# SavaRobotics/FoundationPose

Hardware: AMD Instinct MI355X
Metric: pose-hypotheses/sec (render+refine+score), 252 hyp x 160x160 (higher is better)
Workload: dtype f16

## Files before the change

### foundationpose_amd/csrc/crop.hip

```cpp
#include "common.h"

__device__ __forceinline__ int round_snapped(double x) {
  double f = floor(x), t = x - f;
  if (fabs(t - 0.5) < 1e-4) {
    long long fi = (long long)f;
    return (int)((fi & 1) ? fi + 1 : fi);
  }
  return (int)floor(x + 0.5);
}

__device__ __forceinline__ float frame_at(const float *img, int H, int W, int C, int y, int x, int c) {
  return (y >= 0 && y < H && x >= 0 && x < W) ? img[((size_t)y * W + x) * C + c] : 0.f;
}

__device__ __forceinline__ void crop_observed_px(const CropArgs &a, int b, float mesh_diameter) {
  const int p = blockIdx.x * blockDim.x + threadIdx.x;
  const float *T = a.tf + (size_t)b * 9;
  const float *pose = a.poses + (size_t)b * 16;
  const int H = a.H, W = a.W;
  __shared__ double s_aff[4];
  if (threadIdx.x == 0) {
    const double sx0 = T[0], tx0 = T[2], sy0 = T[4], ty0 = T[5];
    s_aff[0] = (1.0 / sx0) * W / (W - 1.0);
    s_aff[1] = (-tx0 / sx0) * W / (W - 1.0) - 0.5;
    s_aff[2] = (1.0 / sy0) * H / (H - 1.0);
    s_aff[3] = (-ty0 / sy0) * H / (H - 1.0) - 0.5;
  }
  __syncthreads();
  if (p >= a.Ho * a.Wo) return;
  const int j = p / a.Wo, i = p - j * a.Wo;
  const double sx = T[0], tx = T[2], sy = T[4], ty = T[5];
  const double ax = s_aff[0], bx = s_aff[1], ay = s_aff[2], by = s_aff[3];
  const double xd = ax * i + bx, yd = ay * j + by;
  const float x = (float)xd, y = (float)yd;

  float rgb[3];
  {
    float x0f = floorf(x), y0f = floorf(y);
    int x0 = (int)x0f, y0 = (int)y0f, x1 = x0 + 1, y1 = y0 + 1;
    float x1f = x0f + 1.f, y1f = y0f + 1.f;
    float nw = (x1f - x) * (y1f - y), ne = (x - x0f) * (y1f - y), sw = (x1f - x) * (y - y0f), se = (x - x0f) * (y - y0f);
#pragma unroll
    for (int c = 0; c < 3; ++c) {
      float acc = 0.f;
      acc = __fadd_rn(acc, __fmul_rn(frame_at(a.rgb, H, W, 3, y0, x0, c), nw));
      acc = __fadd_rn(acc, __fmul_rn(frame_at(a.rgb, H, W, 3, y0, x1, c), ne));
      acc = __fadd_rn(acc, __fmul_rn(frame_at(a.rgb, H, W, 3, y1, x0, c), sw));
      acc = __fadd_rn(acc, __fmul_rn(frame_at(a.rgb, H, W, 3, y1, x1, c), se));
      rgb[c] = __fdiv_rn(acc, 255.f);
    }
  }
  const int qx = round_snapped(xd), qy = round_snapped(yd);
  const bool q_in = (qx >= 0 && qx < W && qy >= 0 && qy < H);
  float xyz[3] = {0.f, 0.f, 0.f};
  float invalid_thres;
  if (a.mode == 0) {
    invalid_thres = 0.001f;
    if (q_in) {
#pragma unroll
      for (int c = 0; c < 3; ++c) xyz[c] = a.geom[((size_t)qy * W + qx) * 3 + c];
    }
  } else {
    invalid_thres = 0.1f;
    if (q_in) {
      const double cxp = (sx * qx + tx) * a.Wo / (a.Wo - 1.0) - 0.5;
      const double cyp = (sy * qy + ty) * a.Ho / (a.Ho - 1.0) - 0.5;
      const int pi = round_snapped(cxp), pj = round_snapped(cyp);
      float z = 0.f;
      if (pi >= 0 && pi < a.Wo && pj >= 0 && pj < a.Ho) {
        const int rx = round_snapped(ax * pi + bx), ry = round_snapped(ay * pj + by);
        if (rx >= 0 && rx < W && ry >= 0 && ry < H) z = a.geom[(size_t)ry * W + rx];
      }
      const float fx = (float)a.K[0], fy = (float)a.K[4], cx = (float)a.K[2], cy = (float)a.K[5];
      if (!(z < 0.001f)) {
        xyz[0] = __fdiv_rn(__fmul_rn(__fsub_rn((float)qx, cx), z), fx);
        xyz[1] = __fdiv_rn(__fmul_rn(__fsub_rn((float)qy, cy), z), fy);
        xyz[2] = z;
      }
    }
  }
  const bool invalid = xyz[2] < invalid_thres;
  const float radius = __fdiv_rn(mesh_diameter, 2.f);
  const float inv_r = __fdiv_rn(1.f, radius);
  float o6[6] = {rgb[0], rgb[1], rgb[2], 0.f, 0.f, 0.f};
#pragma unroll
  for (int c = 0; c < 3; ++c) {
    float v = __fsub_rn(xyz[c], pose[c * 4 + 3]);
    if (a.normalize_xyz) {
      v = __fmul_rn(v, inv_r);
      if (invalid || fabsf(v) >= 2.f) v = 0.f;
    }
    o6[3 + c] = v;
  }
  if (a.out_fmt == 0) {
    float *out = (float *)a.out + (size_t)b * 6 * a.Ho * a.Wo;
#pragma unroll
    for (int c = 0; c < 6; ++c) out[(size_t)c * a.Ho * a.Wo + p] = o6[c];
  } else {
    half8 hv;
#pragma unroll
    for (int c = 0; c < 6; ++c) hv[c] = (f16)o6[c];
    hv[6] = (f16)0.f;
    hv[7] = (f16)0.f;
    *reinterpret_cast<half8 *>((f16 *)a.out + ((size_t)b * a.Ho * a.Wo + p) * 8) = hv;
  }
}

__global__ __launch_bounds__(256) void crop_observed_kernel(CropArgs a) { crop_observed_px(a, blockIdx.y, a.mesh_diameter); }

struct CropDiameters {
  float d[FP_TRACK_MAX_OBJECTS];
};
__global__ __launch_bounds__(256) void crop_observed_objects_kernel(CropArgs a, CropDiameters t) { crop_observed_px(a, blockIdx.y, t.d[blockIdx.y]); }

int launch_crop_observed(const CropArgs &a, hipStream_t s) {
  FP_REQUIRE(a.mode == 0 || a.mode == 1, "crop_observed: mode must be 0 (refiner) or 1 (scorer)");
  FP_REQUIRE(a.H > 1 && a.W > 1 && a.Ho > 1 && a.Wo > 1, "crop_observed: degenerate image size");
  if (a.N == 0) return FP_OK;
  dim3 grid((a.Ho * a.Wo + 255) / 256, a.N);
  hipLaunchKernelGGL(crop_observed_kernel, grid, dim3(256), 0, s, a);
  FP_CHECK_HIP(hipGetLastError());
  return FP_OK;
}

int launch_crop_observed_objects(const CropArgs &a, const float *diameter, hipStream_t s) {
  FP_REQUIRE(a.mode == 0 || a.mode == 1, "crop_observed: mode must be 0 (refiner) or 1 (scorer)");
  FP_REQUIRE(a.H > 1 && a.W > 1 && a.Ho > 1 && a.Wo > 1, "crop_observed: degenerate image size");
  FP_REQUIRE(a.N >= 0 && a.N <= FP_TRACK_MAX_OBJECTS, "crop_observed: %d objects in one launch (at most %d)", a.N, FP_TRACK_MAX_OBJECTS);
  if (a.N == 0) return FP_OK;
  CropDiameters t;
  memset(&t, 0, sizeof(t));
  for (int b = 0; b < a.N; ++b) t.d[b] = diameter[b];
  hipLaunchKernelGGL(crop_observed_objects_kernel, dim3((a.Ho * a.Wo + 255) / 256, a.N), dim3(256), 0, s, a, t);
  FP_CHECK_HIP(hipGetLastError());
  return FP_OK;
}

__global__ __launch_bounds__(256) void warp_nearest_kernel(const float *__restrict__ src, size_t src_batch_stride, int Hs, int Ws, int C,
                                                           const float *__restrict__ tf, int Ho, int Wo, float *__restrict__ out) {
  const int b = blockIdx.y;
  const int p = blockIdx.x * blockDim.x + threadIdx.x;
  if (p >= Ho * Wo) return;
  const float *T = tf + (size_t)b * 9;
  const double sx = T[0], tx = T[2], sy = T[4], ty = T[5];
  const double ax = (1.0 / sx) * Ws / (Ws - 1.0), bx = (-tx / sx) * Ws / (Ws - 1.0) - 0.5;
  const double ay = (1.0 / sy) * Hs / (Hs - 1.0), by = (-ty / sy) * Hs / (Hs - 1.0) - 0.5;
  const int j = p / Wo, i = p - j * Wo;
  const int qx = round_snapped(ax * i + bx), qy = round_snapped(ay * j + by);
  const bool in = qx >= 0 && qx < Ws && qy >= 0 && qy < Hs;
  const float *s = src + (size_t)b * src_batch_stride + ((size_t)(in ? qy : 0) * Ws + (in ? qx : 0)) * C;
  float *o = out + (size_t)b * C * Ho * Wo + p;
  for (int c = 0; c < C; ++c) o[(size_t)c * Ho * Wo] = in ? s[c] : 0.f;
}

int launch_warp_nearest(const float *src, int src_batch, int Hs, int Ws, int C, const float *tf, int N, int Ho, int Wo, float *out,
                        hipStream_t s) {
  FP_REQUIRE(Hs > 1 && Ws > 1 && Ho > 0 && Wo > 0 && C > 0, "warp_nearest: degenerate image size");
  FP_REQUIRE(src_batch == 1 || src_batch == N, "warp_nearest: the source batch is 1 (broadcast) or N");
  if (N == 0) return FP_OK;
  dim3 grid((Ho * Wo + 255) / 256, N);
  hipLaunchKernelGGL(warp_nearest_kernel, grid, dim3(256), 0, s, src, src_batch == 1 ? (size_t)0 : (size_t)Hs * Ws * C, Hs, Ws, C, tf, Ho,
                     Wo, out);
  FP_CHECK_HIP(hipGetLastError());
  return FP_OK;
}

__global__ void erode_depth_kernel(const float *__restrict__ depth, int H, int W, int radius, float diff_thres, float ratio_thres,
                                   float zfar, float *__restrict__ out) {
  int w = blockIdx.x * blockDim.x + threadIdx.x, h = blockIdx.y * blockDim.y + threadIdx.y;
  if (w >= W || h >= H) return;
  float d_ori = depth[(size_t)h * W + w];
  float bad = 0.f, total = 0.f;
  for (int u = w - radius; u <= w + radius; ++u) {
    if (u < 0 || u >= W) continue;
    for (int v = h - radius; v <= h + radius; ++v) {
      if (v < 0 || v >= H) continue;
      float cur = depth[(size_t)v * W + u];
      total += 1.f;
      if (cur < 0.001f || cur >= zfar || fabsf(cur - d_ori) > diff_thres) bad += 1.f;
    }
  }
  out[(size_t)h * W + w] = (__fdiv_rn(bad, total) > ratio_thres) ? 0.f : d_ori;
}

__global__ void bilateral_depth_kernel(const float *__restrict__ depth, int H, int W, int radius, float zfar, float sigmaD,
                                       float sigmaR, float *__restrict__ out) {
  int w = blockIdx.x * blockDim.x + threadIdx.x, h = blockIdx.y * blockDim.y + threadIdx.y;
  if (w >= W || h >= H) return;
  float mean_depth = 0.f;
  int num_valid = 0;
  for (int u = w - radius; u <= w + radius; ++u) {
    if (u < 0 || u >= W) continue;
    for (int v = h - radius; v <= h + radius; ++v) {
      if (v < 0 || v >= H) continue;
      float cur = depth[(size_t)v * W + u];
      if (cur >= 0.001f && cur < zfar) {
        num_valid += 1;
        mean_depth = __fadd_rn(mean_depth, cur);
      }
    }
  }
  float res = 0.f;
  if (num_valid > 0) {
    mean_depth = __fdiv_rn(mean_depth, (float)num_valid);
    float dc = depth[(size_t)h * W + w];
    float sum_w = 0.f, sum = 0.f;
    const float den_d = __fmul_rn(__fmul_rn(2.f, sigmaD), sigmaD), den_r = __fmul_rn(__fmul_rn(2.f, sigmaR), sigmaR);
    for (int u = w - radius; u <= w + radius; ++u) {
      if (u < 0 || u >= W) continue;
      for (int v = h - radius; v <= h + radius; ++v) {
        if (v < 0 || v >= H) continue;
        float cur = depth[(size_t)v * W + u];
        if (cur >= 0.001f && cur < zfar && fabsf(cur - mean_depth) < 0.01f) {
          float sp = __fdiv_rn(-(float)((u - w) * (u - w) + (h - v) * (h - v)), den_d);
          float df = __fsub_rn(dc, cur);
          float rg = __fdiv_rn(__fmul_rn(df, df), den_r);
          float wt = expf(__fsub_rn(sp, rg));
          sum_w = __fadd_rn(sum_w, wt);
          sum = __fadd_rn(sum, __fmul_rn(wt, cur));
        }
      }
    }
    if (sum_w > 0.f) res = __fdiv_rn(sum, sum_w);
  }
  out[(size_t)h * W + w] = res;
}

__global__ void depth2xyz_kernel(const float *__restrict__ depth, int H, int W, float fx, float fy, float cx, float cy, float zfar,
                                 float *__restrict__ xyz) {
  int w = blockIdx.x * blockDim.x + threadIdx.x, h = blockIdx.y * blockDim.y + threadIdx.y;
  if (w >= W || h >= H) return;
  float z = depth[(size_t)h * W + w];
  float o[3] = {0.f, 0.f, 0.f};
  if (!(z < 0.001f) && !(z > zfar)) {
    o[0] = __fdiv_rn(__fmul_rn(__fsub_rn((float)w, cx), z), fx);
    o[1] = __fdiv_rn(__fmul_rn(__fsub_rn((float)h, cy), z), fy);
    o[2] = z;
  }
  size_t p = ((size_t)h * W + w) * 3;
  xyz[p] = o[0];
  xyz[p + 1] = o[1];
  xyz[p + 2] = o[2];
}

static dim3 grid2d(int H, int W) { return dim3((W + 31) / 32, (H + 7) / 8); }

int launch_erode(const float *d, int H, int W, int radius, float diff_thres, float ratio_thres, float zfar, float *out, hipStream_t s) {
  hipLaunchKernelGGL(erode_depth_kernel, grid2d(H, W), dim3(32, 8), 0, s, d, H, W, radius, diff_thres, ratio_thres, zfar, out);
  FP_CHECK_HIP(hipGetLastError());
  return FP_OK;
}
int launch_bilateral(const float *d, int H, int W, int radius, float zfar, float sigmaD, float sigmaR, float *out, hipStream_t s) {
  hipLaunchKernelGGL(bilateral_depth_kernel, grid2d(H, W), dim3(32, 8), 0, s, d, H, W, radius, zfar, sigmaD, sigmaR, out);
  FP_CHECK_HIP(hipGetLastError());
  return FP_OK;
}
int launch_depth2xyz(const float *d, int H, int W, const double *K, float zfar, float *xyz, hipStream_t s) {
  hipLaunchKernelGGL(depth2xyz_kernel, grid2d(H, W), dim3(32, 8), 0, s, d, H, W, (float)K[0], (float)K[4], (float)K[2], (float)K[5],
                     zfar, xyz);
  FP_CHECK_HIP(hipGetLastError());
  return FP_OK;
}

#define PF_R 2
#define PF_TW 32
#define PF_TH 8
__global__ __launch_bounds__(PF_TW *PF_TH) void depth_prefilter_kernel(const float *__restrict__ depth, int H, int W, float diff_thres,
                                                                       float ratio_thres, float zfar_e, float zfar_b, float sigmaD, float sigmaR,
                                                                       float fx, float fy, float cx, float cy, float zfar_x,
                                                                       float *__restrict__ out, float *__restrict__ xyz,
                                                                       const unsigned char *__restrict__ rgb_u8, float *__restrict__ rgb_f) {
  constexpr int R = PF_R, RW = PF_TW + 4 * R, RH = PF_TH + 4 * R, EW = PF_TW + 2 * R, EH = PF_TH + 2 * R, NTAP = (2 * R + 1) * (2 * R + 1);
  __shared__ float raw[RH][RW + 1], er[EH][EW + 1], sp_tab[NTAP];
  const float OUTSIDE = -__builtin_inff();
  const int tid = threadIdx.y * PF_TW + threadIdx.x, w0 = blockIdx.x * PF_TW, h0 = blockIdx.y * PF_TH;
  if (tid < NTAP) {
    const int du = tid / (2 * R + 1), dv = tid % (2 * R + 1);
    sp_tab[tid] = __fdiv_rn(-(float)((du - R) * (du - R) + (dv - R) * (dv - R)), __fmul_rn(__fmul_rn(2.f, sigmaD), sigmaD));
  }
  for (int i = tid; i < RH * RW; i += PF_TW * PF_TH) {
    const int r = i / RW, c = i - r * RW, h = h0 - 2 * R + r, w = w0 - 2 * R + c;
    raw[r][c] = (h >= 0 && h < H && w >= 0 && w < W) ? depth[(size_t)h * W + w] : OUTSIDE;
  }
  __syncthreads();
  for (int i = tid; i < EH * EW; i += PF_TW * PF_TH) {
    const int r = i / EW, c = i - r * EW;
// ... 172 lines not shown
```

### foundationpose_amd/csrc/raster.hip

```cpp
#include "common.h"
#include "pose_math.h"
#include <cstdlib>
#include <type_traits>

#define RB_THREADS 1024

__device__ __forceinline__ unsigned ordered_key(float z) {
  unsigned b = __float_as_uint(z);
  return (b & 0x80000000u) ? ~b : (b | 0x80000000u);
}

struct Vtx {
  int X, Y;
  float w, zn;
  bool ok;
};

__device__ __forceinline__ Vtx xform_vertex(const float *__restrict__ pos, int v, const float *M, float hw, float hh) {
  float px = pos[v * 3], py = pos[v * 3 + 1], pz = pos[v * 3 + 2];
  float c0 = fmaf(M[0], px, fmaf(M[1], py, fmaf(M[2], pz, M[3])));
  float c1 = fmaf(M[4], px, fmaf(M[5], py, fmaf(M[6], pz, M[7])));
  float c2 = fmaf(M[8], px, fmaf(M[9], py, fmaf(M[10], pz, M[11])));
  float c3 = fmaf(M[12], px, fmaf(M[13], py, fmaf(M[14], pz, M[15])));
  Vtx o;
// ... 180 lines not shown
  __shared__ float sM[16];
  __shared__ float sP[12];
  const int b = blockIdx.x, grp = blockIdx.y;
  const MeshDev &m = a.mesh;
  const uint2 *gA = recA + (size_t)b * m.V;
  const int f0 = grp * Fg, f1 = min(m.F, f0 + Fg);
  for (int i = threadIdx.x; i < S * 3; i += RB_THREADS) cs[i / 3][i % 3] = 0;
  if constexpr (FUSED) {
    if (threadIdx.x == 0) {
      clip_matrix(a, b, a.poses + (size_t)b * 16, sM);
      for (int i = 0; i < 12; ++i) sP[i] = a.poses[(size_t)b * 16 + i];
    }
    __syncthreads();
    for (int v = threadIdx.x; v < m.V; v += RB_THREADS) {
      const VtxRecords q = vertex_records(a, a.mesh, v, sM, sP);
      cl_ldsA[v] = q.a;
      if ((v / RB_THREADS) % G == grp) {
        const size_t r = (size_t)b * m.V + v;
        recC[r] = q.c;
        recA[r] = q.a;
        recB[2 * r] = q.b0;
        recB[2 * r + 1] = q.b1;
      }
    }
  } else if (lds_verts) {
    for (int i = threadIdx.x; i < m.V; i += RB_THREADS) cl_ldsA[i] = gA[i];
  }
  __syncthreads();
  auto getA = [&](int i) -> uint2 { return (FUSED || lds_verts) ? cl_ldsA[i] : gA[i]; };
  const size_t seg = (size_t)G * Fg;
  unsigned *lA = listA + (size_t)b * S * seg + (size_t)grp * Fg, *lB = listB + (size_t)b * S * seg + (size_t)grp * Fg;
  int4 f_n = make_int4(0, 0, 0, 0);
  if (f0 + (int)threadIdx.x < f1) f_n = m.faces4[f0 + threadIdx.x];
  for (int t = f0 + threadIdx.x; t < f1; t += RB_THREADS) {
    const int4 f = f_n;
    if (t + RB_THREADS < f1) f_n = m.faces4[t + RB_THREADS];
    const uint2 a0 = getA(f.x), a1 = getA(f.y), a2 = getA(f.z);
    if (a0.x == RB_A_NONE || a1.x == RB_A_NONE || a2.x == RB_A_NONE) {
      const bool front = (a0.x != RB_A_NONE || __uint_as_float(a0.y) > 0.f) || (a1.x != RB_A_NONE || __uint_as_float(a1.y) > 0.f) ||
                         (a2.x != RB_A_NONE || __uint_as_float(a2.y) > 0.f);
      if (!front) continue;
      for (int sI = 0; sI < S; ++sI) lB[(size_t)sI * seg + atomicAdd(&cs[sI][2], 1)] = (unsigned)t | RB_SLOW;
      continue;
    }
    const int X0 = (short)(a0.x & 0xffffu), Y0 = (int)a0.x >> 16, X1 = (short)(a1.x & 0xffffu), Y1 = (int)a1.x >> 16,
              X2 = (short)(a2.x & 0xffffu), Y2 = (int)a2.x >> 16;
    if ((X1 - X0) * (Y2 - Y0) - (X2 - X0) * (Y1 - Y0) == 0) continue;
    const int xmin = min(X0, min(X1, X2)), xmax = max(X0, max(X1, X2));
    const int ymin = min(Y0, min(Y1, Y2)), ymax = max(Y0, max(Y1, Y2));
    const int ia = max((xmin - 8 + 15) >> 4, 0), ib = min((xmax - 8) >> 4, a.Wo - 1);
    const int ja = max((ymin - 8 + 15) >> 4, 0), jb = min((ymax - 8) >> 4, a.Ho - 1);
    if (ia > ib || ja > jb) continue;
    const int bw = ib - ia + 1;
    for (int sI = ja / strip_rows; sI <= jb / strip_rows; ++sI) {
      const int rows = min(jb, (sI + 1) * strip_rows - 1) - max(ja, sI * strip_rows) + 1;
      const int nc = bw * rows;
      if (nc <= RB_SMALL) lA[(size_t)sI * seg + atomicAdd(&cs[sI][0], 1)] = (unsigned)t;
      else if (nc <= RB_MEDIUM) lA[(size_t)sI * seg + (Fg - 1 - atomicAdd(&cs[sI][1], 1))] = (unsigned)t;
      else lB[(size_t)sI * seg + atomicAdd(&cs[sI][2], 1)] = (unsigned)t;
    }
  }
  __syncthreads();
  for (int i = threadIdx.x; i < S * 3; i += RB_THREADS) count[(((size_t)b * S + i / 3) * G + grp) * 4 + i % 3] = cs[i / 3][i % 3];
}

struct NoObjs {};
struct RenderObjs {
  int n;
  int wg0[FP_TRACK_MAX_OBJECTS + 1], hyp[FP_TRACK_MAX_OBJECTS], n_strips[FP_TRACK_MAX_OBJECTS], strip_rows[FP_TRACK_MAX_OBJECTS];
  float diameter[FP_TRACK_MAX_OBJECTS];
  MeshDev mesh[FP_TRACK_MAX_OBJECTS];
};
template <int MODE, bool SOLO, typename OBJ = NoObjs>
__global__ __launch_bounds__(RB_THREADS) void render_kernel(RenderArgs a, int strip_rows, int n_strips, const int4 *__restrict__ recC,
                                                            const float4 *__restrict__ recB, const uint2 *__restrict__ recA, const int *__restrict__ count,
                                                            const unsigned *__restrict__ listA, const unsigned *__restrict__ listB, int lds_verts, int G, int Fg,
                                                            OBJ t) {
  constexpr bool OBJS = !std::is_same<OBJ, NoObjs>::value;
  extern __shared__ __attribute__((aligned(16))) unsigned long long zbuf[];
  __shared__ float sM[16];
  __shared__ float sP[12];
  __shared__ int covn;
  __shared__ int scnt[3];
  const int L = xcd_remap(blockIdx.x, gridDim.x);
  int b, strip;
  const MeshDev *mp = &a.mesh;
  float obj_diameter = 0.f;
  if constexpr (OBJS) {
    int o = 0;
    while (o + 1 < t.n && L >= t.wg0[o + 1]) ++o;
    b = t.hyp[o], strip = L - t.wg0[o];
    strip_rows = t.strip_rows[o], n_strips = t.n_strips[o];
    mp = &t.mesh[o];
    obj_diameter = t.diameter[o];
  } else {
    b = L / n_strips, strip = L % n_strips;
  }
  const int Ho = a.Ho, Wo = a.Wo;
  const int row0 = strip * strip_rows;
  const int row1 = min(Ho, row0 + strip_rows);
  const int npix = (row1 - row0) * Wo;
  const float *pose = a.poses + (size_t)b * 16;
  const MeshDev &m = *mp;
  const uint2 *gA = recA + (size_t)b * m.V;
  unsigned short *covq = reinterpret_cast<unsigned short *>(zbuf + (size_t)strip_rows * Wo);
  uint2 *ldsA = reinterpret_cast<uint2 *>(reinterpret_cast<char *>(covq) + ((((size_t)strip_rows * Wo * 2) + 15) & ~(size_t)15));
  unsigned short *soloA = reinterpret_cast<unsigned short *>(ldsA + ((m.V + 1) & ~1));
  unsigned short *soloB = soloA + ((m.F + 7) & ~7);

  if (threadIdx.x == 0) {
    clip_matrix(a, b, pose, sM);
    covn = 0;
    if constexpr (SOLO) {
      for (int i = 0; i < 12; ++i) sP[i] = pose[i];
      scnt[0] = scnt[1] = scnt[2] = 0;
    }
  }
  for (int i = threadIdx.x; i < npix; i += RB_THREADS) zbuf[i] = ~0ull;
  if constexpr (SOLO) {
    __syncthreads();
    for (int v = threadIdx.x; v < m.V; v += RB_THREADS) ldsA[v] = (a.dbg & 64) ? make_uint2(RB_A_NONE, 0u) : vertex_records(a, m, v, sM, sP).a;
    __syncthreads();
    auto file_face = [&](int t, const int4 &f) {
      const uint2 a0 = ldsA[f.x], a1 = ldsA[f.y], a2 = ldsA[f.z];
      if (a0.x == RB_A_NONE || a1.x == RB_A_NONE || a2.x == RB_A_NONE) {
        const bool front = (a0.x != RB_A_NONE || __uint_as_float(a0.y) > 0.f) || (a1.x != RB_A_NONE || __uint_as_float(a1.y) > 0.f) ||
                           (a2.x != RB_A_NONE || __uint_as_float(a2.y) > 0.f);
        if (front) soloB[atomicAdd(&scnt[2], 1)] = (unsigned short)t;
        return;
      }
      const int X0 = (short)(a0.x & 0xffffu), Y0 = (int)a0.x >> 16, X1 = (short)(a1.x & 0xffffu), Y1 = (int)a1.x >> 16,
                X2 = (short)(a2.x & 0xffffu), Y2 = (int)a2.x >> 16;
      if ((X1 - X0) * (Y2 - Y0) - (X2 - X0) * (Y1 - Y0) == 0) return;
      const int xmin = min(X0, min(X1, X2)), xmax = max(X0, max(X1, X2));
      const int ymin = min(Y0, min(Y1, Y2)), ymax = max(Y0, max(Y1, Y2));
      const int ia = max((xmin - 8 + 15) >> 4, 0), ib = min((xmax - 8) >> 4, Wo - 1);
      const int ja = max((ymin - 8 + 15) >> 4, row0), jb = min((ymax - 8) >> 4, row1 - 1);
      if (ia > ib || ja > jb) return;
      const int nc = (ib - ia + 1) * (jb - ja + 1);
      if (nc <= RB_SMALL) soloA[atomicAdd(&scnt[0], 1)] = (unsigned short)t;
      else if (nc <= RB_MEDIUM) soloA[m.F - 1 - atomicAdd(&scnt[1], 1)] = (unsigned short)t;
      else soloB[atomicAdd(&scnt[2], 1)] = (unsigned short)t;
    };
    const int F_do = (a.dbg & 32) ? 0 : m.F;
    for (int t0 = threadIdx.x; t0 < F_do; t0 += 4 * RB_THREADS) {
      int4 fq[4];
#pragma unroll
      for (int u = 0; u < 4; ++u) fq[u] = m.faces4[min(t0 + u * RB_THREADS, m.F - 1)];
#pragma unroll
      for (int u = 0; u < 4; ++u)
        if (t0 + u * RB_THREADS < F_do) file_face(t0 + u * RB_THREADS, fq[u]);
    }
  } else if (lds_verts) {
    for (int i = threadIdx.x; i < m.V; i += RB_THREADS) ldsA[i] = gA[i];
  }
  __syncthreads();

  const float *M = sM;
  const float hw = 0.5f * (float)Wo, hh = 0.5f * (float)Ho;
  const int4 *vc = recC + (size_t)b * m.V;
  const float4 *vbB = recB + 2 * (size_t)b * m.V;
  auto getA = [&](int i) -> uint2 { return (SOLO || lds_verts) ? ldsA[i] : gA[i]; };
  auto getC = [&](int i) -> int4 {
    if constexpr (SOLO) return vertex_records(a, m, i, sM, sP).c;
    else return vc[i];
  };
  auto unpack = [](const int4 &q) -> Vtx {
    Vtx o;
    o.X = q.x;
    o.Y = q.y;
    o.zn = __int_as_float(q.z);
    o.w = __int_as_float(q.w);
    o.ok = q.x != (int)0x80000000;
    return o;
  };
  const int lane = threadIdx.x & 63, wave = threadIdx.x >> 6;
  if constexpr (SOLO) G = 1, Fg = m.F;
  for (int grp = 0; grp < G; ++grp) {
  const int *cnt = SOLO ? scnt : count + (((size_t)b * n_strips + strip) * G + grp) * 4;
  const int n_small = (a.dbg & 4) ? 0 : cnt[0], n_med = (a.dbg & 4) ? 0 : cnt[1], n_b = (a.dbg & 20) ? 0 : cnt[2];
  const unsigned *lA = listA + ((size_t)b * n_strips + strip) * G * Fg + (size_t)grp * Fg, *lB = listB + ((size_t)b * n_strips + strip) * G * Fg + (size_t)grp * Fg;
  auto entryA = [&](int i) -> int { return SOLO ? (int)soloA[i] : (int)lA[i]; };
  auto entryB = [&](int i) -> int { return SOLO ? (int)soloB[i] : (int)(lB[i] & ~RB_SLOW); };

  {
    const int n_a = n_small + n_med;
    auto entry = [&](int e) -> int { return e < n_small ? entryA(e) : entryA(Fg - 1 - (e - n_small)); };
    int t_n = 0;
    int4 f_n = make_int4(0, 0, 0, 0);
    if ((int)threadIdx.x < n_a) {
      t_n = entry(threadIdx.x);
      f_n = m.faces4[t_n];
    }
    for (int e = threadIdx.x; e < n_a; e += RB_THREADS) {
      const int t = t_n;
      const int4 f = f_n;
      if (e + RB_THREADS < n_a) {
        t_n = entry(e + RB_THREADS);
        f_n = m.faces4[t_n];
      }
      if (a.dbg & 1) continue;
      const uint2 a0 = getA(f.x), a1 = getA(f.y), a2 = getA(f.z);
      const int X0 = (short)(a0.x & 0xffffu), Y0 = (int)a0.x >> 16, X1 = (short)(a1.x & 0xffffu), Y1 = (int)a1.x >> 16,
                X2 = (short)(a2.x & 0xffffu), Y2 = (int)a2.x >> 16;
      int area = (X1 - X0) * (Y2 - Y0) - (X2 - X0) * (Y1 - Y0);
      const int xmin = min(X0, min(X1, X2)), xmax = max(X0, max(X1, X2));
      const int ymin = min(Y0, min(Y1, Y2)), ymax = max(Y0, max(Y1, Y2));
      int ia = (xmin - 8 + 15) >> 4, ib = (xmax - 8) >> 4, ja = (ymin - 8 + 15) >> 4, jb = (ymax - 8) >> 4;
      ia = max(ia, 0);
      ja = max(ja, row0);
      ib = min(ib, Wo - 1);
      jb = min(jb, row1 - 1);
      const int sg = area > 0 ? 1 : -1;
      area *= sg;
      const int dx0 = sg * (X2 - X1), dy0 = sg * (Y2 - Y1);
      const int dx1 = sg * (X0 - X2), dy1 = sg * (Y0 - Y2);
      const int dx2 = sg * (X1 - X0), dy2 = sg * (Y1 - Y0);
      const bool tl0 = (dy0 > 0) || (dy0 == 0 && dx0 < 0);
      const bool tl1 = (dy1 > 0) || (dy1 == 0 && dx1 < 0);
      const bool tl2 = (dy2 > 0) || (dy2 == 0 && dx2 < 0);
      const float fa = (float)area;
      const float z0 = __uint_as_float(a0.y), z1 = __uint_as_float(a1.y), z2 = __uint_as_float(a2.y);
      for (int j = ja; j <= jb; ++j) {
        const int Py = 16 * j + 8;
        for (int i = ia; i <= ib; ++i) {
          const int Px = 16 * i + 8;
          const int e0 = dx0 * (Py - Y1) - dy0 * (Px - X1);
          const int e1 = dx1 * (Py - Y2) - dy1 * (Px - X2);
          const int e2 = dx2 * (Py - Y0) - dy2 * (Px - X0);
          if (!((e0 > 0 || (e0 == 0 && tl0)) && (e1 > 0 || (e1 == 0 && tl1)) && (e2 > 0 || (e2 == 0 && tl2)))) continue;
          const float b0 = (float)e0 / fa, b1 = (float)e1 / fa, b2 = (float)e2 / fa;
          const float zp = fmaf(b2, z2, fmaf(b1, z1, b0 * z0));
          if (!(zp >= -1.f && zp <= 1.f)) continue;
          const unsigned long long key = ((unsigned long long)ordered_key(zp) << 32) | (unsigned)t;
          atomicMin(&zbuf[(j - row0) * Wo + i], key);
        }
      }
    }
  }
  constexpr int CHB = 4;
  for (int base = wave * CHB; base < n_b; base += (RB_THREADS / 64) * CHB) {
    int my_t = 0;
    int4 my_f = make_int4(0, 0, 0, 0), my_c0 = my_f, my_c1 = my_f, my_c2 = my_f;
    if (lane < CHB && base + lane < n_b) {
      my_t = entryB(base + lane);
      my_f = m.faces4[my_t];
      my_c0 = getC(my_f.x), my_c1 = getC(my_f.y), my_c2 = getC(my_f.z);
    }
    const int cntw = min(CHB, n_b - base);
    for (int q = 0; q < cntw; ++q) {
      auto bc4 = [&](const int4 &x) -> int4 {
        return make_int4(__builtin_amdgcn_readlane(x.x, q), __builtin_amdgcn_readlane(x.y, q), __builtin_amdgcn_readlane(x.z, q),
                         __builtin_amdgcn_readlane(x.w, q));
      };
      const int t = __builtin_amdgcn_readlane(my_t, q);
      const int4 f = bc4(my_f);
      const Vtx v0 = unpack(bc4(my_c0)), v1 = unpack(bc4(my_c1)), v2 = unpack(bc4(my_c2));
      if (!(v0.ok && v1.ok && v2.ok)) {
        if (!(v0.w > 0.f || v1.w > 0.f || v2.w > 0.f)) continue;
        float c[3][4];
        const int fi3[3] = {f.x, f.y, f.z};
#pragma unroll
        for (int k = 0; k < 3; ++k) clip_coords(m.pos, fi3[k], M, c[k]);
        const ClipTri T = clip_setup(c, hw, hh);
        if (!T.valid) continue;
        for (int p = lane; p < npix; p += 64) {
          const int jl = p / Wo, i = p - jl * Wo;
          float l[3], zp;
          if (!clip_eval(T, i, row0 + jl, l, &zp)) continue;
          const unsigned long long key = ((unsigned long long)ordered_key(zp) << 32) | (unsigned)t;
          atomicMin(&zbuf[p], key);
        }
        continue;
      }
      const long long X0 = v0.X, Y0 = v0.Y, X1 = v1.X, Y1 = v1.Y, X2 = v2.X, Y2 = v2.Y;
      long long area = (X1 - X0) * (Y2 - Y0) - (X2 - X0) * (Y1 - Y0);
      if (area == 0) continue;
      const long long sg = area > 0 ? 1 : -1;
      area *= sg;
      const long long xmin = min(X0, min(X1, X2)), xmax = max(X0, max(X1, X2));
      const long long ymin = min(Y0, min(Y1, Y2)), ymax = max(Y0, max(Y1, Y2));
      long long ia = (xmin - 8 + 15) >> 4, ib = (xmax - 8) >> 4, ja = (ymin - 8 + 15) >> 4, jb = (ymax - 8) >> 4;
      ia = max(ia, 0ll);
      ja = max(ja, (long long)row0);
      ib = min(ib, (long long)Wo - 1);
      jb = min(jb, (long long)row1 - 1);
      if (ia > ib || ja > jb) continue;
      const long long dx0 = sg * (X2 - X1), dy0 = sg * (Y2 - Y1);
      const long long dx1 = sg * (X0 - X2), dy1 = sg * (Y0 - Y2);
      const long long dx2 = sg * (X1 - X0), dy2 = sg * (Y1 - Y0);
      const bool tl0 = (dy0 > 0) || (dy0 == 0 && dx0 < 0);
      const bool tl1 = (dy1 > 0) || (dy1 == 0 && dx1 < 0);
      const bool tl2 = (dy2 > 0) || (dy2 == 0 && dx2 < 0);
      const float fa = (float)area;
      const int bw = (int)(ib - ia + 1), ncand = bw * (int)(jb - ja + 1);
      for (int k = lane; k < ncand; k += 64) {
        const int jj = k / bw;
        const long long i = ia + (k - jj * bw), j = ja + jj;
        const long long Px = 16 * i + 8, Py = 16 * j + 8;
        const long long e0 = dx0 * (Py - Y1) - dy0 * (Px - X1);
        const long long e1 = dx1 * (Py - Y2) - dy1 * (Px - X2);
        const long long e2 = dx2 * (Py - Y0) - dy2 * (Px - X0);
        if (!((e0 > 0 || (e0 == 0 && tl0)) && (e1 > 0 || (e1 == 0 && tl1)) && (e2 > 0 || (e2 == 0 && tl2)))) continue;
        const float b0 = (float)e0 / fa, b1 = (float)e1 / fa, b2 = (float)e2 / fa;
        const float zp = fmaf(b2, v2.zn, fmaf(b1, v1.zn, b0 * v0.zn));
        if (!(zp >= -1.f && zp <= 1.f)) continue;
        const unsigned long long key = ((unsigned long long)ordered_key(zp) << 32) | (unsigned)t;
// ... 431 lines not shown
```

Before: 7457.

## Precompute per-row/column crop axis tables in LDS and batch gathers; vectorize vertex LDS copy

The crop kernel now tiles the output into row bands and column tiles. Per-column and per-row affine results (bilinear weights, snapped indices, and the scorer's round-trip depth index) are computed once into shared memory, where before every pixel recomputed them in double precision. Each thread issues gathers for two pixels before finishing them, and 3-channel loads use 12-byte memcpy with 32-bit offsets. Separately, the raster kernel copies vertex records into LDS with 16-byte vector loads when aligned, and the band height shrinks when there are few hypotheses to keep enough workgroups.

```diff
diff --git a/foundationpose_amd/csrc/crop.hip b/foundationpose_amd/csrc/crop.hip
--- a/foundationpose_amd/csrc/crop.hip
+++ b/foundationpose_amd/csrc/crop.hip
@@ -9,85 +9,128 @@
   return (int)floor(x + 0.5);
 }
 
-__device__ __forceinline__ float frame_at(const float *img, int H, int W, int C, int y, int x, int c) {
-  return (y >= 0 && y < H && x >= 0 && x < W) ? img[((size_t)y * W + x) * C + c] : 0.f;
-}
-
-__device__ __forceinline__ void crop_observed_px(const CropArgs &a, int b, float mesh_diameter) {
-  const int p = blockIdx.x * blockDim.x + threadIdx.x;
-  const float *T = a.tf + (size_t)b * 9;
-  const float *pose = a.poses + (size_t)b * 16;
-  const int H = a.H, W = a.W;
-  __shared__ double s_aff[4];
+struct CropAxis {
+  float w0, w1;
+  int p0, q, r;
+};
+__device__ __forceinline__ CropAxis crop_axis(double c0, double c1, int idx, double s, double t, int n_src, int n_out, int mode) {
+  const double xd = c0 * idx + c1;
+  const float x = (float)xd;
+  const float x0f = floorf(x), x1f = x0f + 1.f;
+  CropAxis e;
+  e.w0 = x1f - x;
+  e.w1 = x - x0f;
+  e.p0 = (int)x0f;
+  const int q = round_snapped(xd);
+  const bool in = q >= 0 && q < n_src;
+  e.q = in ? q : -1;
+  e.r = -1;
+  if (mode == 1 && in) {
+    const double cp = (s * q + t) * n_out / (n_out - 1.0) - 0.5;
+    const int pi = round_snapped(cp);
+    if (pi >= 0 && pi < n_out) {
+      const int r = round_snapped(c0 * pi + c1);
+      if (r >= 0 && r < n_src) e.r = r;
+    }
+  }
+  return e;
+}
+
+__device__ __forceinline__ void crop_affine(const CropArgs &a, const float *T, double *s_aff) {
   if (threadIdx.x == 0) {
     const double sx0 = T[0], tx0 = T[2], sy0 = T[4], ty0 = T[5];
-    s_aff[0] = (1.0 / sx0) * W / (W - 1.0);
-    s_aff[1] = (-tx0 / sx0) * W / (W - 1.0) - 0.5;
-    s_aff[2] = (1.0 / sy0) * H / (H - 1.0);
-    s_aff[3] = (-ty0 / sy0) * H / (H - 1.0) - 0.5;
+    s_aff[0] = (1.0 / sx0) * a.W / (a.W - 1.0);
+    s_aff[1] = (-tx0 / sx0) * a.W / (a.W - 1.0) - 0.5;
+    s_aff[2] = (1.0 / sy0) * a.H / (a.H - 1.0);
+    s_aff[3] = (-ty0 / sy0) * a.H / (a.H - 1.0) - 0.5;
   }
   __syncthreads();
-  if (p >= a.Ho * a.Wo) return;
-  const int j = p / a.Wo, i = p - j * a.Wo;
-  const double sx = T[0], tx = T[2], sy = T[4], ty = T[5];
-  const double ax = s_aff[0], bx = s_aff[1], ay = s_aff[2], by = s_aff[3];
-  const double xd = ax * i + bx, yd = ay * j + by;
-  const float x = (float)xd, y = (float)yd;
-
+}
+
+struct CropTaps {
+  float c[3][4];
+  float g[3];
+};
+__device__ __forceinline__ void crop_load3(const float *img, unsigned off, bool ok, float &v0, float &v1, float &v2) {
+  float v[3];
+  __builtin_memcpy(v, img + (ok ? off : 0u), 12);
+  v0 = ok ? v[0] : 0.f, v1 = ok ? v[1] : 0.f, v2 = ok ? v[2] : 0.f;
+}
+__device__ __forceinline__ CropTaps crop_gather(const CropArgs &a, const CropAxis &cx, const CropAxis &cy) {
+  const unsigned H = a.H, W = a.W;
+  CropTaps t;
+  const unsigned x0 = (unsigned)cx.p0, y0 = (unsigned)cy.p0, x1 = x0 + 1u, y1 = y0 + 1u;
+  const bool vx0 = x0 < W, vx1 = x1 < W, vy0 = y0 < H, vy1 = y1 < H;
+  const unsigned o00 = (y0 * W + x0) * 3u, o10 = o00 + W * 3u;
+  crop_load3(a.rgb, o00, vy0 && vx0, t.c[0][0], t.c[1][0], t.c[2][0]);
+  crop_load3(a.rgb, o00 + 3u, vy0 && vx1, t.c[0][1], t.c[1][1], t.c[2][1]);
+  crop_load3(a.rgb, o10, vy1 && vx0, t.c[0][2], t.c[1][2], t.c[2][2]);
+  crop_load3(a.rgb, o10 + 3u, vy1 && vx1, t.c[0][3], t.c[1][3], t.c[2][3]);
+  const bool q_in = cx.q >= 0 && cy.q >= 0;
+  if (a.mode == 0) {
+    crop_load3(a.geom, ((unsigned)cy.q * W + (unsigned)cx.q) * 3u, q_in, t.g[0], t.g[1], t.g[2]);
+  } else {
+    const bool r_in = q_in && cx.r >= 0 && cy.r >= 0;
+    const float z = a.geom[r_in ? (unsigned)cy.r * W + (unsigned)cx.r : 0u];
+    t.g[0] = r_in ? z : 0.f;
+    t.g[1] = t.g[2] = 0.f;
+  }
+  return t;
+}
+
+struct CropConsts {
+  float t[3], inv_r, fx, fy, cx, cy;
+};
+__device__ __forceinline__ CropConsts crop_consts(const CropArgs &a, int b, float mesh_diameter) {
+  const float *pose = a.poses + (size_t)b * 16;
+  CropConsts k;
+  k.t[0] = pose[3], k.t[1] = pose[7], k.t[2] = pose[11];
+  k.inv_r = __fdiv_rn(1.f, __fdiv_rn(mesh_diameter, 2.f));
+  k.fx = (float)a.K[0], k.fy = (float)a.K[4], k.cx = (float)a.K[2], k.cy = (float)a.K[5];
+  return k;
+}
+__device__ __forceinline__ void crop_finish(const CropArgs &a, int b, const CropConsts &k, int i, int j, const CropAxis &cx, const CropAxis &cy,
+                                            const CropTaps &t) {
+  const int p = j * a.Wo + i;
   float rgb[3];
   {
-    float x0f = floorf(x), y0f = floorf(y);
-    int x0 = (int)x0f, y0 = (int)y0f, x1 = x0 + 1, y1 = y0 + 1;
-    float x1f = x0f + 1.f, y1f = y0f + 1.f;
-    float nw = (x1f - x) * (y1f - y), ne = (x - x0f) * (y1f - y), sw = (x1f - x) * (y - y0f), se = (x - x0f) * (y - y0f);
+    const float nw = cx.w0 * cy.w0, ne = cx.w1 * cy.w0, sw = cx.w0 * cy.w1, se = cx.w1 * cy.w1;
 #pragma unroll
     for (int c = 0; c < 3; ++c) {
       float acc = 0.f;
-      acc = __fadd_rn(acc, __fmul_rn(frame_at(a.rgb, H, W, 3, y0, x0, c), nw));
-      acc = __fadd_rn(acc, __fmul_rn(frame_at(a.rgb, H, W, 3, y0, x1, c), ne));
-      acc = __fadd_rn(acc, __fmul_rn(frame_at(a.rgb, H, W, 3, y1, x0, c), sw));
-      acc = __fadd_rn(acc, __fmul_rn(frame_at(a.rgb, H, W, 3, y1, x1, c), se));
+      acc = __fadd_rn(acc, __fmul_rn(t.c[c][0], nw));
+      acc = __fadd_rn(acc, __fmul_rn(t.c[c][1], ne));
+      acc = __fadd_rn(acc, __fmul_rn(t.c[c][2], sw));
+      acc = __fadd_rn(acc, __fmul_rn(t.c[c][3], se));
       rgb[c] = __fdiv_rn(acc, 255.f);
     }
   }
-  const int qx = round_snapped(xd), qy = round_snapped(yd);
-  const bool q_in = (qx >= 0 && qx < W && qy >= 0 && qy < H);
+  const int qx = cx.q, qy = cy.q;
+  const bool q_in = qx >= 0 && qy >= 0;
   float xyz[3] = {0.f, 0.f, 0.f};
   float invalid_thres;
   if (a.mode == 0) {
     invalid_thres = 0.001f;
-    if (q_in) {
-#pragma unroll
-      for (int c = 0; c < 3; ++c) xyz[c] = a.geom[((size_t)qy * W + qx) * 3 + c];
-    }
+#pragma unroll
+    for (int c = 0; c < 3; ++c) xyz[c] = t.g[c];
   } else {
     invalid_thres = 0.1f;
     if (q_in) {
-      const double cxp = (sx * qx + tx) * a.Wo / (a.Wo - 1.0) - 0.5;
-      const double cyp = (sy * qy + ty) * a.Ho / (a.Ho - 1.0) - 0.5;
-      const int pi = round_snapped(cxp), pj = round_snapped(cyp);
-      float z = 0.f;
-      if (pi >= 0 && pi < a.Wo && pj >= 0 && pj < a.Ho) {
-        const int rx = round_snapped(ax * pi + bx), ry = round_snapped(ay * pj + by);
-        if (rx >= 0 && rx < W && ry >= 0 && ry < H) z = a.geom[(size_t)ry * W + rx];
-      }
-      const float fx = (float)a.K[0], fy = (float)a.K[4], cx = (float)a.K[2], cy = (float)a.K[5];
+      const float z = t.g[0];
       if (!(z < 0.001f)) {
-        xyz[0] = __fdiv_rn(__fmul_rn(__fsub_rn((float)qx, cx), z), fx);
-        xyz[1] = __fdiv_rn(__fmul_rn(__fsub_rn((float)qy, cy), z), fy);
+        xyz[0] = __fdiv_rn(__fmul_rn(__fsub_rn((float)qx, k.cx), z), k.fx);
+        xyz[1] = __fdiv_rn(__fmul_rn(__fsub_rn((float)qy, k.cy), z), k.fy);
         xyz[2] = z;
       }
     }
   }
   const bool invalid = xyz[2] < invalid_thres;
-  const float radius = __fdiv_rn(mesh_diameter, 2.f);
-  const float inv_r = __fdiv_rn(1.f, radius);
   float o6[6] = {rgb[0], rgb[1], rgb[2], 0.f, 0.f, 0.f};
 #pragma unroll
   for (int c = 0; c < 3; ++c) {
-    float v = __fsub_rn(xyz[c], pose[c * 4 + 3]);
+    float v = __fsub_rn(xyz[c], k.t[c]);
     if (a.normalize_xyz) {
-      v = __fmul_rn(v, inv_r);
+      v = __fmul_rn(v, k.inv_r);
       if (invalid || fabsf(v) >= 2.f) v = 0.f;
     }
     o6[3 + c] = v;
@@ -106,19 +149,96 @@
   }
 }
 
-__global__ __launch_bounds__(256) void crop_observed_kernel(CropArgs a) { crop_observed_px(a, blockIdx.y, a.mesh_diameter); }
+#define CROP_TW 512
+#define CROP_BH 16
+#define CROP_U 2
+template <bool TABLES, int U>
+__device__ __forceinline__ void crop_observed_wg(const CropArgs &a, int b, float mesh_diameter, int band_rows) {
+  const float *T = a.tf + (size_t)b * 9;
+  const double sx = T[0], tx = T[2], sy = T[4], ty = T[5];
+  if constexpr (!TABLES) {
+    __shared__ double s_aff[4];
+    crop_affine(a, T, s_aff);
+    const double ax = s_aff[0], bx = s_aff[1], ay = s_aff[2], by = s_aff[3];
+    const int p = blockIdx.x * blockDim.x + threadIdx.x;
+    if (p >= a.Ho * a.Wo) return;
+    const int j = p / a.Wo, i = p - j * a.Wo;
+    const CropAxis cx = crop_axis(ax, bx, i, sx, tx, a.W, a.Wo, a.mode), cy = crop_axis(ay, by, j, sy, ty, a.H, a.Ho, a.mode);
+    crop_finish(a, b, crop_consts(a, b, mesh_diameter), i, j, cx, cy, crop_gather(a, cx, cy));
+  } else {
+    __shared__ CropAxis s_col[CROP_TW], s_row[CROP_BH];
+    const int n_ct = (a.Wo + CROP_TW - 1) / CROP_TW;
+    const int band = blockIdx.x / n_ct, ct = blockIdx.x - band * n_ct;
+    const int i0 = ct * CROP_TW, cw = min(CROP_TW, a.Wo - i0);
+    const int j0 = band * band_rows, rows = min(band_rows, a.Ho - j0);
+    for (int e = threadIdx.x; e < cw + rows; e += 256) {
+      if (e < cw) {
+        const double ax = (1.0 / sx) * a.W / (a.W - 1.0), bx = (-tx / sx) * a.W / (a.W - 1.0) - 0.5;
+        s_col[e] = crop_axis(ax, bx, i0 + e, sx, tx, a.W, a.Wo, a.mode);
+      } else {
+        const double ay = (1.0 / sy) * a.H / (a.H - 1.0), by = (-ty / sy) * a.H / (a.H - 1.0) - 0.5;
+        s_row[e - cw] = crop_axis(ay, by, j0 + e - cw, sy, ty, a.H, a.Ho, a.mode);
+      }
+    }
+    __syncthreads();
+    const int dj = 256 / cw, di = 256 - dj * cw;
+    int jl = threadIdx.x / cw, il = threadIdx.x - jl * cw;
+    const CropConsts k = crop_consts(a, b, mesh_diameter);
+    while (jl < rows) {
+      int pi[U], pj[U];
+      CropTaps taps[U];
+#pragma unroll
+      for (int u = 0; u < U; ++u) {
+        pi[u] = il, pj[u] = jl;
+        if (jl < rows) taps[u] = crop_gather(a, s_col[il], s_row[jl]);
+        il += di;
+        jl += dj;
+        if (il >= cw) il -= cw, ++jl;
+      }
+#pragma unroll
+      for (int u = 0; u < U; ++u)
+        if (pj[u] < rows) crop_finish(a, b, k, i0 + pi[u], j0 + pj[u], s_col[pi[u]], s_row[pj[u]], taps[u]);
+    }
+  }
+}
+
+template <bool TABLES, int U>
+__global__ __launch_bounds__(256) void crop_observed_kernel(CropArgs a, int band_rows) {
+  crop_observed_wg<TABLES, U>(a, blockIdx.y, a.mesh_diameter, band_rows);
+}
 
 struct CropDiameters {
   float d[FP_TRACK_MAX_OBJECTS];
 };
-__global__ __launch_bounds__(256) void crop_observed_objects_kernel(CropArgs a, CropDiameters t) { crop_observed_px(a, blockIdx.y, t.d[blockIdx.y]); }
+template <bool TABLES, int U>
+__global__ __launch_bounds__(256) void crop_observed_objects_kernel(CropArgs a, CropDiameters t, int band_rows) {
+  crop_observed_wg<TABLES, U>(a, blockIdx.y, t.d[blockIdx.y], band_rows);
+}
+
+static bool crop_grid(const CropArgs &a, unsigned *wgs, int *band_rows) {
+  static const bool per_pixel = fp_env_set("FP_CROP_PER_PIXEL");
+  if (per_pixel) {
+    *wgs = (unsigned)((a.Ho * a.Wo + 255) / 256);
+    *band_rows = 0;
+    return false;
+  }
+  const int n_ct = (a.Wo + CROP_TW - 1) / CROP_TW;
+  int bh = CROP_BH;
+  while (bh > 2 && (size_t)a.N * ((a.Ho + bh - 1) / bh) * n_ct < 1024) bh /= 2;
+  *wgs = (unsigned)(((a.Ho + bh - 1) / bh) * n_ct);
+  *band_rows = bh;
+  return true;
+}
 
 int launch_crop_observed(const CropArgs &a, hipStream_t s) {
   FP_REQUIRE(a.mode == 0 || a.mode == 1, "crop_observed: mode must be 0 (refiner) or 1 (scorer)");
   FP_REQUIRE(a.H > 1 && a.W > 1 && a.Ho > 1 && a.Wo > 1, "crop_observed: degenerate image size");
+  FP_REQUIRE((size_t)a.H * a.W * 3 < ((size_t)1 << 31), "crop_observed: a %d x %d frame is beyond the kernel's 32-bit element offsets", a.H, a.W);
   if (a.N == 0) return FP_OK;
-  dim3 grid((a.Ho * a.Wo + 255) / 256, a.N);
-  hipLaunchKernelGGL(crop_observed_kernel, grid, dim3(256), 0, s, a);
+  unsigned wgs;
+  int band_rows;
+  if (crop_grid(a, &wgs, &band_rows)) hipLaunchKernelGGL((crop_observed_kernel<true, CROP_U>), dim3(wgs, a.N), dim3(256), 0, s, a, band_rows);
+  else hipLaunchKernelGGL((crop_observed_kernel<false, 1>), dim3(wgs, a.N), dim3(256), 0, s, a, band_rows);
   FP_CHECK_HIP(hipGetLastError());
   return FP_OK;
 }
@@ -126,12 +246,16 @@
 int launch_crop_observed_objects(const CropArgs &a, const float *diameter, hipStream_t s) {
   FP_REQUIRE(a.mode == 0 || a.mode == 1, "crop_observed: mode must be 0 (refiner) or 1 (scorer)");
   FP_REQUIRE(a.H > 1 && a.W > 1 && a.Ho > 1 && a.Wo > 1, "crop_observed: degenerate image size");
+  FP_REQUIRE((size_t)a.H * a.W * 3 < ((size_t)1 << 31), "crop_observed: a %d x %d frame is beyond the kernel's 32-bit element offsets", a.H, a.W);
   FP_REQUIRE(a.N >= 0 && a.N <= FP_TRACK_MAX_OBJECTS, "crop_observed: %d objects in one launch (at most %d)", a.N, FP_TRACK_MAX_OBJECTS);
   if (a.N == 0) return FP_OK;
   CropDiameters t;
   memset(&t, 0, sizeof(t));
   for (int b = 0; b < a.N; ++b) t.d[b] = diameter[b];
-  hipLaunchKernelGGL(crop_observed_objects_kernel, dim3((a.Ho * a.Wo + 255) / 256, a.N), dim3(256), 0, s, a, t);
+  unsigned wgs;
+  int band_rows;
+  if (crop_grid(a, &wgs, &band_rows)) hipLaunchKernelGGL((crop_observed_objects_kernel<true, CROP_U>), dim3(wgs, a.N), dim3(256), 0, s, a, t, band_rows);
+  else hipLaunchKernelGGL((crop_observed_objects_kernel<false, 1>), dim3(wgs, a.N), dim3(256), 0, s, a, t, band_rows);
   FP_CHECK_HIP(hipGetLastError());
   return FP_OK;
 }
diff --git a/foundationpose_amd/csrc/raster.hip b/foundationpose_amd/csrc/raster.hip
--- a/foundationpose_amd/csrc/raster.hip
+++ b/foundationpose_amd/csrc/raster.hip
@@ -356,7 +356,13 @@
         if (t0 + u * RB_THREADS < F_do) file_face(t0 + u * RB_THREADS, fq[u]);
     }
   } else if (lds_verts) {
-    for (int i = threadIdx.x; i < m.V; i += RB_THREADS) ldsA[i] = gA[i];
+    if ((((size_t)gA | (size_t)ldsA) & 15) == 0 && !(m.V & 1) && !(a.dbg & 128)) {
+      const uint4 *g4 = reinterpret_cast<const uint4 *>(gA);
+      uint4 *l4 = reinterpret_cast<uint4 *>(ldsA);
+      for (int i = threadIdx.x; i < m.V / 2; i += RB_THREADS) l4[i] = g4[i];
+    } else {
+      for (int i = threadIdx.x; i < m.V; i += RB_THREADS) ldsA[i] = gA[i];
+    }
   }
   __syncthreads();
 
```

Result: no change. 7490 (median of 6 runs) (+0.5%).
